# zju3dv/LoFTR

Hardware: AMD Instinct MI355X
Metric: image-pairs/sec @640x480 indoor-ds (higher is better)
Workload: dtype f32; 1 GPU; batch=8 640x480 synthetic grayscale pairs per GPU, indoor_ds dual-softmax (BASELINE configs[1]), full LoFTR.forward = ResNet-FPN backbone (HIP implicit-GEMM / patch convolutions incl. the 7x7 stem) + HIP matching path; weights=seeded random init (no checkpoint on the box), conf_matrix_materialised=True, match_type=dual_softmax, global_batch=8, parallelism=dp1 (pairs sharded; RCCL all-gather of match counts)

## Files before the change

loftr_amd/csrc/common.h:

```cpp
#pragma once
#include <hip/hip_runtime.h>
#include <stdint.h>
#include <stddef.h>
#include "../../include/loftr_hip.h"

typedef float f32x16 __attribute__((ext_vector_type(16)));
typedef float f32x4 __attribute__((ext_vector_type(4)));
typedef float f32x2 __attribute__((ext_vector_type(2)));

#define LOFTR_NEG_INF (-1e9f)

#define LOFTR_CHECK_ARG(cond) do { if (!(cond)) return LOFTR_ERR_BAD_ARG; } while (0)
#define LOFTR_CHECK_LAUNCH() do { if (hipGetLastError() != hipSuccess) return LOFTR_ERR_LAUNCH; } while (0)

#ifdef __HIP_DEVICE_COMPILE__
#define LOFTR_NO_PACKED_FP32 __attribute__((target("no-packed-fp32-ops")))
#else
#define LOFTR_NO_PACKED_FP32
#endif

__host__ __device__ static inline int ceil_div(int a, int b) { return (a + b - 1) / b; }
static inline size_t align_up(size_t x, size_t a) { return (x + a - 1) / a * a; }

enum LoftrTimedKernel {
// ... 13 lines not shown
  LOFTR_T_ENCODER_X = 13,
  LOFTR_T_FINE_PAIR = 14,
  LOFTR_T_COUNT = 15
};
enum LoftrDebugKey {
  LOFTR_DBG_ENCODER_SCHEDULE = 0,
  LOFTR_DBG_CONV_PERSIST_CAP,
  LOFTR_DBG_WGRAD_CHUNK,
  LOFTR_DBG_REDUCE_TALL,
  LOFTR_DBG_PCT_GRID,
  LOFTR_DBG_PCT_SKIP,
  LOFTR_DBG_PCT_QUOTA,
  LOFTR_DBG_CONV_DUO,
  LOFTR_DBG_CONV_PATCH,
  LOFTR_DBG_CONV_REM,
  LOFTR_DBG_COUNT
};
int loftr_debug_value(int key);
extern unsigned g_loftr_timing_mask;
extern int g_loftr_range_check;
void loftr_timing_mark(int id, hipStream_t st, bool end);
struct TimedLaunch {
  int id; hipStream_t st; bool on;
  TimedLaunch(int id_, hipStream_t st_) : id(id_), st(st_), on((g_loftr_timing_mask >> id_) & 1u) {
    if (on) loftr_timing_mark(id, st, false);
  }
  ~TimedLaunch() { if (on) loftr_timing_mark(id, st, true); }
};

constexpr int NUM_XCD = 8;
// ... 98 lines not shown
```

loftr_amd/csrc/fine_fused.hip:

```cpp
#include "linear.h"

#ifdef LOFTR_FINE_PROBE
__device__ long long* g_fine_probe = nullptr;
#define FFX_STAMP(i_) { const long long t__ = wall_clock64(); pacc[i_] += t__ - pt__; pt__ = t__; }
#else
#define FFX_STAMP(i_)
#endif
#ifndef FFX_PROBE_READS
#define FFX_PROBE_READS 1
#endif
#ifndef FFX_PROBE_DMA
#define FFX_PROBE_DMA 1
#endif
#ifndef FFX_PROBE_BARRIER
#define FFX_PROBE_BARRIER 1
#endif
namespace {
namespace ffx {
constexpr int W = 4, STAGE = 16 * 1024, BLK = 4096, NST = 6, DMA_PER_WAVE = 4;
constexpr int PPC = 8 + 8 + 24, NCALL = 4, NPANEL = PPC * NCALL;
constexpr int T_QS = 0, T_KS = 128, T_VS = 256, T_MS = 384, T_W0S = 512, T_W2S = 768, T_G1 = 896, T_B1 = 1024, T_G2 = 1152,
              T_B2 = 1280, T_LAYER = 1408;
constexpr int OFF_TAB = NST * STAGE, OFF_KSUM = OFF_TAB + 2 * T_LAYER * 4;
constexpr int OFF_KV = OFF_KSUM + W * 512;
constexpr int OFF_DESC = OFF_KV + W * 8192;
constexpr int LDS_BYTES = OFF_DESC + NPANEL * 16;
static_assert(LDS_BYTES <= 160 * 1024, "one workgroup per CU");

struct Args {
  float* f0; float* f1;
  int M, T;
  const sp_t* wq[2]; const sp_t* wk[2]; const sp_t* wv[2]; const sp_t* wm[2]; const sp_t* w0[2]; const sp_t* w2[2];
  const float* sq[2]; const float* sk[2]; const float* sv[2]; const float* sm[2]; const float* s0[2]; const float* s2[2];
  const float* g1[2]; const float* b1[2]; const float* g2[2]; const float* b2[2];
  float attn_eps, ln_eps;
};

typedef __attribute__((address_space(3))) void* lds_ptr_t;
typedef const __attribute__((address_space(1))) void* gbl_ptr_t;

__device__ __forceinline__ void swap_halves(uint32_t& a, uint32_t& b) {
  const auto r = __builtin_amdgcn_permlane32_swap(a, b, false, false);
// ... 39 lines not shown
__device__ __forceinline__ float wave_absmax16(const float (&v)[16]) {
  float m = 0.f;
#pragma unroll
  for (int r = 0; r < 16; ++r) m = fmaxf(m, fabsf(v[r]));
  m = half_max(m);
  return fmaxf(m, swap32(m));
}
__device__ __forceinline__ void pack8(const float (&v)[8], h16x8& fh, h16x8& fl) {
  uint32_t hi[4], lo[4];
#pragma unroll
  for (int e = 0; e < 4; ++e) sp_pack2(v[2 * e], v[2 * e + 1], hi[e], lo[e]);
  fh = __builtin_bit_cast(h16x8, u32x4{hi[0], hi[1], hi[2], hi[3]});
  fl = __builtin_bit_cast(h16x8, u32x4{lo[0], lo[1], lo[2], lo[3]});
}

__device__ __forceinline__ float kv_tile(const f32x16& kacc, const f32x16& vacc, float ksc, float vsc, int T, int g, int li,
                                         unsigned ksum_ad, unsigned kv_ad) {
  float kk[16], vv[16], ksum = 0.f;
#pragma unroll
  for (int r = 0; r < 16; ++r) {
    const bool ok = (r & 3) + 8 * (r >> 2) + 4 * g < T;
    const float kx = kacc[r] * ksc;
    kk[r] = ok ? (kx > 0.f ? kx + 1.f : __expf(kx)) : 0.f;
    vv[r] = ok ? vacc[r] * vsc : 0.f;
    ksum += kk[r];
  }
  ksum += swap32(ksum);
  float v_inv;
  const float v_sc = pow2_lift(wave_absmax16(vv), v_inv);
#pragma unroll
// ... 18 lines not shown
  }
  float kvv[16];
#pragma unroll
  for (int r = 0; r < 16; ++r) kvv[r] = kv[r];
  float kv_inv;
  const float kv_sc = pow2_lift(wave_absmax16(kvv), kv_inv);
#pragma unroll
  for (int r = 0; r < 16; ++r) kvv[r] *= kv_sc;
  h16x8 fh[2], fl[2];
  pack_panel(kvv, fh, fl);
  const u32x4 mh = __builtin_bit_cast(u32x4, li < 16 ? fh[0] : fh[1]), ml = __builtin_bit_cast(u32x4, li < 16 ? fl[0] : fl[1]);
  asm volatile("ds_write_b128 %0, %1\n\tds_write_b128 %0, %2 offset:1024" :: "v"(kv_ad), "v"(mh), "v"(ml) : "memory");
  return v_inv * kv_inv;
}

__global__ __launch_bounds__(W * 64, 1) void fine_pair_kernel(Args a) {
  __shared__ __attribute__((aligned(16))) char lds[LDS_BYTES];
  const int lane = threadIdx.x & 63, wave = threadIdx.x >> 6, g = lane >> 5, li = lane & 31;
  const int T = a.T;
  const long m = (long)blockIdx.x * W + wave;
  const bool live = m < a.M;
  const long mc = live ? m : a.M - 1;
  float* tab = reinterpret_cast<float*>(lds + OFF_TAB);
  const unsigned ksum_addr = (unsigned)(size_t)(lds_ptr_t)(lds + OFF_KSUM + wave * 512);
  const float* ksum_tab = reinterpret_cast<const float*>(lds + OFF_KSUM + wave * 512);
  const unsigned kv_addr = (unsigned)(size_t)(lds_ptr_t)(lds + OFF_KV + wave * 8192);
  const char* kv_tab = lds + OFF_KV + wave * 8192 + lane * 16;

  for (int f = threadIdx.x; f < 256; f += W * 64) {
#pragma unroll
    for (int l = 0; l < 2; ++l) {
      float* tl = tab + l * T_LAYER;
      tl[T_W0S + f] = a.s0[l][f];
      if (f < 128) {
        tl[T_QS + f] = a.sq[l][f]; tl[T_KS + f] = a.sk[l][f]; tl[T_VS + f] = a.sv[l][f]; tl[T_MS + f] = a.sm[l][f];
        tl[T_W2S + f] = a.s2[l][f];
        tl[T_G1 + f] = a.g1[l][f]; tl[T_B1 + f] = a.b1[l][f]; tl[T_G2 + f] = a.g2[l][f]; tl[T_B2 + f] = a.b2[l][f];
      }
    }
  }
  h16x8 wah[8], wal[8], wbh[8], wbl[8];
  float wa_sc, wa_inv, wb_sc, wb_inv;
  {
    const long row = (mc * T + min(li, T - 1)) * 128;
    const f32x4* p0 = reinterpret_cast<const f32x4*>(a.f0 + row);
    const f32x4* p1 = reinterpret_cast<const f32x4*>(a.f1 + row);
    f32x4 ua[16], ub[16];
    float ma = 0.f, mb = 0.f;
#pragma unroll
    for (int i = 0; i < 16; ++i) {
      ua[i] = p0[4 * (i >> 1) + 2 * g + (i & 1)]; ub[i] = p1[4 * (i >> 1) + 2 * g + (i & 1)];
#pragma unroll
      for (int e = 0; e < 4; ++e) { ma = fmaxf(ma, fabsf(ua[i][e])); mb = fmaxf(mb, fabsf(ub[i][e])); }
    }
    ma = half_max(ma); ma = fmaxf(ma, swap32(ma)); mb = half_max(mb); mb = fmaxf(mb, swap32(mb));
    wa_sc = pow2_lift(ma, wa_inv); wb_sc = pow2_lift(mb, wb_inv);
#pragma unroll
    for (int ks = 0; ks < 8; ++ks) {
      const f32x4 u0 = ua[2 * ks] * wa_sc, u1 = ua[2 * ks + 1] * wa_sc, v0 = ub[2 * ks] * wb_sc, v1 = ub[2 * ks + 1] * wb_sc;
      const float xa[8] = {u0[0], u0[1], u0[2], u0[3], u1[0], u1[1], u1[2], u1[3]};
      const float xb[8] = {v0[0], v0[1], v0[2], v0[3], v1[0], v1[1], v1[2], v1[3]};
      pack8(xa, wah[ks], wal[ks]);
      pack8(xb, wbh[ks], wbl[ks]);
    }
  }

  unsigned off128[4];
#pragma unroll
  for (int oct = 0; oct < 4; ++oct) {
    const unsigned ro = oct * 8 + (lane >> 3), ch = ((lane & 7) ^ ((oct * 4 + (lane >> 4)) & 7)) << 2;
    off128[oct] = (ro * 128 + ch) * 4;
  }
  const unsigned rl512 = (unsigned)(lane >> 3) * 512u;
  const int wave_s = __builtin_amdgcn_readfirstlane(wave);
  for (int p = threadIdx.x; p < NPANEL; p += W * 64) {
    const int c = p / PPC, q = p - c * PPC, l = c >> 1;
    int off, pitch = 128, mat, kt = 0;
    if (q < 8) { mat = (q & 1) ? 2 : 1; off = (q >> 1) * 32 * 128; }
    else if (q < 16) { const int t = (q - 8) >> 1; if (q & 1) { mat = 3; off = t * 32; kt = 1; } else { mat = 0; off = t * 32 * 128; } }
    else { const int hp = (q - 16) / 3, i = (q - 16) - 3 * hp; pitch = 256;
           if (i == 2) { mat = 5; off = hp * 32; kt = 1; } else { mat = 4; off = hp * 32 * 256 + i * 128; } }
    const sp_t* mp = mat == 0 ? a.wq[l] : mat == 1 ? a.wk[l] : mat == 2 ? a.wv[l] : mat == 3 ? a.wm[l] : mat == 4 ? a.w0[l] : a.w2[l];
    const unsigned long long ad = (unsigned long long)(size_t)(mp + off);
    reinterpret_cast<int4*>(lds + OFF_DESC)[p] = make_int4((int)(unsigned)ad, (int)(unsigned)(ad >> 32), pitch, kt);
  }
#define FFX_ISSUE(p_)                                                                                      \
  {                                                                                                        \
    const int p__ = (p_);                                                                                  \
    const int4 d__ = reinterpret_cast<const int4*>(lds + OFF_DESC)[p__];                                   \
    const unsigned lo__ = (unsigned)__builtin_amdgcn_readfirstlane(d__.x), hi__ = (unsigned)__builtin_amdgcn_readfirstlane(d__.y); \
    const int pitch__ = __builtin_amdgcn_readfirstlane(d__.z), kt__ = __builtin_amdgcn_readfirstlane(d__.w);        \
    const unsigned long long wo__ = (unsigned long long)(kt__ ? wave_s * 32 * pitch__ : wave_s * 32) * 4ull;    \
    const char* base__ = reinterpret_cast<const char*>((size_t)((((unsigned long long)hi__ << 32) | lo__) + wo__)); \
    char* st__ = lds + (p__ % NST) * STAGE + wave_s * BLK;                                                 \
    const unsigned w256__ = pitch__ == 256 ? 1u : 0u;                                                      \
    _Pragma("unroll") for (int oct__ = 0; oct__ < 4; ++oct__)                                              \
      __builtin_amdgcn_global_load_lds((gbl_ptr_t)(base__ + (size_t)(w256__ * (unsigned)(oct__ * 4096)) + (off128[oct__] + w256__ * rl512)), \
                                       (lds_ptr_t)(st__ + oct__ * 1024), 16, 0, 0);                        \
  }
#define FFX_BEGIN(p_)                                                                                      \
  {                                                                                                        \
    const int rem__ = NPANEL - 1 - (p_);                                                                   \
    if (!FFX_PROBE_DMA) LOFTR_WAITCNT_VM(0);                                                               \
    else if (rem__ >= 4) LOFTR_WAITCNT_VM(4 * DMA_PER_WAVE);                                                    \
    else if (rem__ == 3) LOFTR_WAITCNT_VM(3 * DMA_PER_WAVE);                                               \
    else if (rem__ == 2) LOFTR_WAITCNT_VM(2 * DMA_PER_WAVE);                                               \
    else if (rem__ == 1) LOFTR_WAITCNT_VM(1 * DMA_PER_WAVE);                                               \
    else LOFTR_WAITCNT_VM(0);                                                                              \
    if (FFX_PROBE_BARRIER) __builtin_amdgcn_s_barrier();                                                   \
    if (FFX_PROBE_DMA && (p_) + NST - 1 < NPANEL) FFX_ISSUE((p_) + NST - 1);                                                \
  }
  const int a_off = lds_chunk_off(li, g);
#define FFX_RD(st_, blk_, odd_, lo_) (*reinterpret_cast<const h16x8*>((st_) + (blk_) * BLK + (a_off ^ (((odd_) ? 32 : 0) | ((lo_) ? 64 : 0)))))
#define FFX_USE(a_, b_, c_, d_) asm volatile("" :: "v"(a_), "v"(b_), "v"(c_), "v"(d_))
#define FFX_UNITS(st_, BLK0_, ODD0_, BLK1_, ODD1_, M1_, M2_, M3_, M4_, M5_, M6_)                           \
  {                                                                                                        \
    h16x8 ah__ = FFX_RD(st_, BLK0_(0), ODD0_(0), 0), al__ = FFX_RD(st_, BLK0_(0), ODD0_(0), 1);            \
    h16x8 bh__ = FFX_RD(st_, BLK1_(0), ODD1_(0), 0), bl__ = FFX_RD(st_, BLK1_(0), ODD1_(0), 1);            \
    _Pragma("unroll") for (int u = 0; u < 4; ++u) {                                                        \
      FFX_USE(ah__, al__, bh__, bl__);                                                                     \
      __builtin_amdgcn_sched_barrier(0);                                                                   \
      h16x8 nah__ = ah__, nal__ = al__, nbh__ = bh__, nbl__ = bl__;                                        \
      M1_;                                                                                                 \
      __builtin_amdgcn_sched_barrier(0);                                                                   \
      if (FFX_PROBE_READS && u + 1 < 4) { nah__ = FFX_RD(st_, BLK0_(u + 1), ODD0_(u + 1), 0); nal__ = FFX_RD(st_, BLK0_(u + 1), ODD0_(u + 1), 1); } \
      __builtin_amdgcn_sched_barrier(0);                                                                   \
      M2_;                                                                                                 \
      __builtin_amdgcn_sched_barrier(0);                                                                   \
      if (FFX_PROBE_READS && u + 1 < 4) { nbh__ = FFX_RD(st_, BLK1_(u + 1), ODD1_(u + 1), 0); nbl__ = FFX_RD(st_, BLK1_(u + 1), ODD1_(u + 1), 1); } \
      __builtin_amdgcn_sched_barrier(0);                                                                   \
      M3_; M4_; M5_; M6_;                                                                                  \
      __builtin_amdgcn_sched_barrier(0);                                                                   \
      ah__ = nah__; al__ = nal__; bh__ = nbh__; bl__ = nbl__;                                              \
    }                                                                                                      \
  }
#define FFX_MF(A_, B_, C_) C_ = __builtin_amdgcn_mfma_f32_32x32x16_f16(A_, B_, C_, 0, 0, 0)
#define FFX_ID(u_) (u_)
#define FFX_ZERO(u_) 0
#define FFX_ONE(u_) 1
#define FFX_RPANEL(st_, xh_, xl_, acc_)                                                                    \
  FFX_UNITS(st_, FFX_ID, FFX_ZERO, FFX_ID, FFX_ONE,                                                        \
            FFX_MF(ah__, xl_[2 * u], acc_), FFX_MF(al__, xh_[2 * u], acc_), FFX_MF(ah__, xh_[2 * u], acc_), \
            FFX_MF(bh__, xl_[2 * u + 1], acc_), FFX_MF(bl__, xh_[2 * u + 1], acc_), FFX_MF(bh__, xh_[2 * u + 1], acc_))
#define FFX_TPANEL(st_, xh_, xl_, acc_)                                                                    \
  FFX_UNITS(st_, FFX_ID, FFX_ZERO, FFX_ID, FFX_ONE,                                                        \
            FFX_MF(xh_[2 * u], al__, acc_), FFX_MF(xl_[2 * u], ah__, acc_), FFX_MF(xh_[2 * u], ah__, acc_), \
            FFX_MF(xh_[2 * u + 1], bl__, acc_), FFX_MF(xl_[2 * u + 1], bh__, acc_), FFX_MF(xh_[2 * u + 1], bh__, acc_))
#define FFX_KB0(u_) (2 * ((u_) >> 1))
#define FFX_KB1(u_) (2 * ((u_) >> 1) + 1)
#define FFX_KODD(u_) ((u_) & 1)
#define FFX_KPANEL(st_, fh_, fl_, out_)                                                                    \
  FFX_UNITS(st_, FFX_KB0, FFX_KODD, FFX_KB1, FFX_KODD,                                                     \
            FFX_MF(ah__, fl_[u & 1], out_[2 * (u >> 1)]), FFX_MF(bh__, fl_[u & 1], out_[2 * (u >> 1) + 1]), \
            FFX_MF(al__, fh_[u & 1], out_[2 * (u >> 1)]), FFX_MF(bl__, fh_[u & 1], out_[2 * (u >> 1) + 1]), \
            FFX_MF(ah__, fh_[u & 1], out_[2 * (u >> 1)]), FFX_MF(bh__, fh_[u & 1], out_[2 * (u >> 1) + 1]))

  LOFTR_WAITCNT_VM(0);
  __syncthreads();
#pragma unroll
  for (int p = 0; p < NST - 1; ++p) FFX_ISSUE(p);

#ifdef LOFTR_FINE_PROBE
  long long pacc[8] = {0, 0, 0, 0, 0, 0, 0, 0};
  const long long pstart__ = wall_clock64();
  long long pt__ = pstart__;
#endif
  const int fq = 4 * g;
  const float S = (float)T, inv_s = 1.f / (float)T;
  const h16x8 zero8 = __builtin_bit_cast(h16x8, u32x4{0u, 0u, 0u, 0u});
  f32x16 acc, acc2;
  f32x16 big[4];

#pragma unroll 1
  for (int c = 0; c < NCALL; ++c) {
    const int p0 = c * PPC;
    const float* tl = tab + (c >> 1) * T_LAYER;
    const bool self = c < 2;
    const float src_sc = self ? wa_sc : wb_sc, src_inv = self ? wa_inv : wb_inv;
    float kvi[4] = {1.f, 1.f, 1.f, 1.f};
#define FFX_KV_LOOP(SH_, SL_)                                                                              \
    _Pragma("unroll 1") for (int t = 0; t < 4; ++t) {                                                      \
      const int p = p0 + 2 * t;                                                                            \
      FFX_BEGIN(p);                                                                                        \
      if (live) {                                                                                          \
        _Pragma("unroll") for (int r = 0; r < 16; ++r) acc[r] = 0.f;                                       \
        FFX_TPANEL(lds + (p % NST) * STAGE, SH_, SL_, acc);        \
      }                                                                                                    \
      FFX_BEGIN(p + 1);                                                                                    \
      if (live) {                                                                                          \
        _Pragma("unroll") for (int r = 0; r < 16; ++r) acc2[r] = 0.f;                                      \
        FFX_TPANEL(lds + ((p + 1) % NST) * STAGE, SH_, SL_, acc2);                             \
        const float inv__ = kv_tile(acc, acc2, tl[T_KS + 32 * t + li] * src_inv, tl[T_VS + 32 * t + li] * inv_s * src_inv, T, g, li, \
                                    ksum_addr + (unsigned)((32 * t + li) * 4), kv_addr + (unsigned)(t * 2048 + lane * 16));  \
        kvi[0] = kvi[1]; kvi[1] = kvi[2]; kvi[2] = kvi[3]; kvi[3] = inv__;                                 \
      }                                                                                                    \
    }
    FFX_STAMP(0)
    if (self) { FFX_KV_LOOP(wah, wal) } else { FFX_KV_LOOP(wbh, wbl) }
#undef FFX_KV_LOOP
    FFX_STAMP(1)
    asm volatile("s_waitcnt lgkmcnt(0)" ::: "memory");
#pragma unroll
    for (int j = 0; j < 4; ++j)
#pragma unroll
      for (int r = 0; r < 16; ++r) big[j][r] = 0.f;
#pragma unroll 1
    for (int t = 0; t < 4; ++t) {
      const int p = p0 + 8 + 2 * t;
      FFX_BEGIN(p);
      h16x8 mah[2], mal[2];
      if (live) {
#pragma unroll
        for (int r = 0; r < 16; ++r) acc[r] = 0.f;
        FFX_RPANEL(lds + (p % NST) * STAGE, wah, wal, acc);
        float v[16], den0 = 0.f, den1 = 0.f;
#pragma unroll
        for (int q = 0; q < 4; ++q) {
          const f32x4 ws = *reinterpret_cast<const f32x4*>(tl + T_QS + 32 * t + fq + 8 * q);
          const f32x4 ks4 = *reinterpret_cast<const f32x4*>(ksum_tab + 32 * t + fq + 8 * q);
#pragma unroll
          for (int e = 0; e < 4; ++e) {
            float x = acc[4 * q + e] * (ws[e] * wa_inv);
            x = x > 0.f ? x + 1.f : __expf(x);
            v[4 * q + e] = x;
            if (q < 2) den0 = fmaf(x, ks4[e], den0); else den1 = fmaf(x, ks4[e], den1);
          }
        }
        den0 += swap32(den0); den1 += swap32(den1);
        const float z0 = S * __builtin_amdgcn_rcpf(den0 + a.attn_eps), z1 = S * __builtin_amdgcn_rcpf(den1 + a.attn_eps);
// ... 11 lines not shown
        const h16x8 kvh0 = *reinterpret_cast<const h16x8*>(kv_tab + t * 2048), kvl0 = *reinterpret_cast<const h16x8*>(kv_tab + t * 2048 + 1024);
        const h16x8 a0h = li < 16 ? kvh0 : zero8, a0l = li < 16 ? kvl0 : zero8;
        const h16x8 a1h = li < 16 ? zero8 : kvh0, a1l = li < 16 ? zero8 : kvl0;
        f32x16 at;
#pragma unroll
        for (int r = 0; r < 16; ++r) at[r] = 0.f;
        FFX_MF(a0h, ql[0], at); FFX_MF(a0l, qh[0], at); FFX_MF(a0h, qh[0], at);
        FFX_MF(a1h, ql[1], at); FFX_MF(a1l, qh[1], at); FFX_MF(a1h, qh[1], at);
        kvi[0] = kvi[1]; kvi[1] = kvi[2]; kvi[2] = kvi[3];
        float av[16];
#pragma unroll
        for (int r = 0; r < 16; ++r) av[r] = at[r] * undo;
        pack_panel(av, mah, mal);
      }
      FFX_BEGIN(p + 1);
      if (live) FFX_KPANEL(lds + ((p + 1) % NST) * STAGE, mah, mal, big);
    }
    FFX_STAMP(2)
    h16x8 mh[8], ml[8];
    if (live) {
      float s = 0.f;
#pragma unroll
      for (int j = 0; j < 4; ++j)
#pragma unroll
        for (int q = 0; q < 4; ++q) {
          const f32x4 ws = *reinterpret_cast<const f32x4*>(tl + T_MS + 32 * j + fq + 8 * q);
#pragma unroll
          for (int e = 0; e < 4; ++e) { big[j][4 * q + e] *= ws[e] * (4.f * src_inv); s += big[j][4 * q + e]; }
        }
      s += swap32(s);
      const float mean = s * (1.f / 128.f);
      float m2 = 0.f;
#pragma unroll
      for (int j = 0; j < 4; ++j)
#pragma unroll
        for (int r = 0; r < 16; ++r) { const float d = big[j][r] - mean; m2 = fmaf(d, d, m2); }
      m2 += swap32(m2);
      const float rstd = rsqrtf(m2 * (1.f / 128.f) + a.ln_eps);
#pragma unroll
      for (int j = 0; j < 4; ++j) {
        float y[16];
#pragma unroll
        for (int q = 0; q < 4; ++q) {
          const f32x4 ga = *reinterpret_cast<const f32x4*>(tl + T_G1 + 32 * j + fq + 8 * q);
          const f32x4 be = *reinterpret_cast<const f32x4*>(tl + T_B1 + 32 * j + fq + 8 * q);
#pragma unroll
          for (int e = 0; e < 4; ++e) y[4 * q + e] = (big[j][4 * q + e] - mean) * rstd * ga[e] + be[e];
        }
        h16x8 fh[2], fl[2];
        pack_panel(y, fh, fl);
        mh[2 * j] = fh[0]; mh[2 * j + 1] = fh[1]; ml[2 * j] = fl[0]; ml[2 * j + 1] = fl[1];
      }
    }
#pragma unroll
    for (int j = 0; j < 4; ++j)
#pragma unroll
      for (int r = 0; r < 16; ++r) big[j][r] = 0.f;
    FFX_STAMP(3)
#pragma unroll 1
    for (int hp = 0; hp < 8; ++hp) {
      const int p = p0 + 16 + 3 * hp;
      h16x8 hh[2], hl[2];
      FFX_BEGIN(p);
      if (live) {
#pragma unroll
        for (int r = 0; r < 16; ++r) acc[r] = 0.f;
        FFX_RPANEL(lds + (p % NST) * STAGE, wah, wal, acc);
      }
      FFX_BEGIN(p + 1);
      if (live) {
#pragma unroll
        for (int r = 0; r < 16; ++r) acc2[r] = 0.f;
        FFX_RPANEL(lds + ((p + 1) % NST) * STAGE, mh, ml, acc2);
        float v[16];
#pragma unroll
        for (int q = 0; q < 4; ++q) {
          const f32x4 ws = *reinterpret_cast<const f32x4*>(tl + T_W0S + 32 * hp + fq + 8 * q);
#pragma unroll
          for (int e = 0; e < 4; ++e) v[4 * q + e] = fmaxf(fmaf(acc[4 * q + e], wa_inv, acc2[4 * q + e]) * ws[e], 0.f);
        }
        pack_panel(v, hh, hl);
      }
      FFX_BEGIN(p + 2);
      if (live) FFX_KPANEL(lds + ((p + 2) % NST) * STAGE, hh, hl, big);
    }
    FFX_STAMP(4)
    if (live) {
      float* orow = ((c & 1) ? a.f1 : a.f0) + (mc * T + min(li, T - 1)) * 128;
      f32x4 xres[16];
#pragma unroll
      for (int j = 0; j < 4; ++j)
#pragma unroll
        for (int q = 0; q < 4; ++q) xres[4 * j + q] = *reinterpret_cast<const f32x4*>(orow + 32 * j + fq + 8 * q);
      float s = 0.f;
#pragma unroll
      for (int j = 0; j < 4; ++j)
#pragma unroll
        for (int q = 0; q < 4; ++q) {
          const f32x4 ws = *reinterpret_cast<const f32x4*>(tl + T_W2S + 32 * j + fq + 8 * q);
#pragma unroll
          for (int e = 0; e < 4; ++e) { big[j][4 * q + e] *= ws[e]; s += big[j][4 * q + e]; }
        }
      s += swap32(s);
      const float mean = s * (1.f / 128.f);
      float m2 = 0.f;
#pragma unroll
      for (int j = 0; j < 4; ++j)
#pragma unroll
        for (int r = 0; r < 16; ++r) { const float d = big[j][r] - mean; m2 = fmaf(d, d, m2); }
      m2 += swap32(m2);
      const float rstd = rsqrtf(m2 * (1.f / 128.f) + a.ln_eps);
      const bool store = li < T;
      float y[4][16], ym = 0.f;
#pragma unroll
      for (int j = 0; j < 4; ++j) {
#pragma unroll
        for (int q = 0; q < 4; ++q) {
          const f32x4 ga = *reinterpret_cast<const f32x4*>(tl + T_G2 + 32 * j + fq + 8 * q);
          const f32x4 be = *reinterpret_cast<const f32x4*>(tl + T_B2 + 32 * j + fq + 8 * q);
          f32x4 o;
#pragma unroll
          for (int e = 0; e < 4; ++e) {
            o[e] = xres[4 * j + q][e] + ((big[j][4 * q + e] - mean) * rstd * ga[e] + be[e]);
            y[j][4 * q + e] = o[e];
            ym = fmaxf(ym, fabsf(o[e]));
          }
          if (store) *reinterpret_cast<f32x4*>(orow + 32 * j + fq + 8 * q) = o;
        }
      }
      ym = half_max(ym); ym = fmaxf(ym, swap32(ym));
      wa_sc = pow2_lift(ym, wa_inv);
#pragma unroll
      for (int j = 0; j < 4; ++j) {
#pragma unroll
        for (int r = 0; r < 16; ++r) y[j][r] *= wa_sc;
        h16x8 fh[2], fl[2];
        pack_panel(y[j], fh, fl);
        wah[2 * j] = fh[0]; wah[2 * j + 1] = fh[1]; wal[2 * j] = fl[0]; wal[2 * j + 1] = fl[1];
      }
    }
#pragma unroll
    for (int ks = 0; ks < 8; ++ks) {
      const h16x8 th = wah[ks], tlo = wal[ks];
      wah[ks] = wbh[ks]; wal[ks] = wbl[ks]; wbh[ks] = th; wbl[ks] = tlo;
    }
    { const float ts = wa_sc, ti = wa_inv; wa_sc = wb_sc; wa_inv = wb_inv; wb_sc = ts; wb_inv = ti; }
    FFX_STAMP(5)
  }
#ifdef LOFTR_FINE_PROBE
  if (g_fine_probe && lane == 0) {
    long long* o = g_fine_probe + ((long)blockIdx.x * W + wave) * 8;
    for (int i = 0; i < 6; ++i) o[i] = pacc[i];
    o[6] = pstart__; o[7] = wall_clock64();
  }
#endif
#undef FFX_ISSUE
#undef FFX_BEGIN
#undef FFX_RD
#undef FFX_USE
#undef FFX_UNITS
#undef FFX_MF
#undef FFX_ID
#undef FFX_ZERO
#undef FFX_ONE
#undef FFX_RPANEL
#undef FFX_TPANEL
#undef FFX_KB0
#undef FFX_KB1
#undef FFX_KODD
#undef FFX_KPANEL
}
}
}

#ifdef LOFTR_FINE_PROBE
extern "C" int loftr_fine_probe_buffer(void* buf) {
  long long* b = (long long*)buf;
  return hipMemcpyToSymbol(HIP_SYMBOL(g_fine_probe), &b, sizeof(b)) == hipSuccess ? LOFTR_OK : LOFTR_ERR_LAUNCH;
}
#endif

int launch_fine_pair(const FinePairArgs& p, hipStream_t st) {
  if (p.C != 128 || p.T < 1 || p.T > 32 || p.M <= 0) return LOFTR_ERR_UNSUPPORTED;
  ffx::Args a{};
  a.f0 = p.f0; a.f1 = p.f1; a.M = p.M; a.T = p.T; a.attn_eps = p.attn_eps; a.ln_eps = p.ln_eps;
  for (int l = 0; l < 2; ++l) {
    a.wq[l] = p.wq[l]; a.wk[l] = p.wk[l]; a.wv[l] = p.wv[l]; a.wm[l] = p.wm[l]; a.w0[l] = p.w0[l]; a.w2[l] = p.w2[l];
    a.sq[l] = p.sq[l]; a.sk[l] = p.sk[l]; a.sv[l] = p.sv[l]; a.sm[l] = p.sm[l]; a.s0[l] = p.s0[l]; a.s2[l] = p.s2[l];
    a.g1[l] = p.g1[l]; a.b1[l] = p.b1[l]; a.g2[l] = p.g2[l]; a.b2[l] = p.b2[l];
    if (!a.wq[l] || !a.sq[l] || !a.sk[l] || !a.sv[l] || !a.sm[l] || !a.s0[l] || !a.s2[l]) return LOFTR_ERR_UNSUPPORTED;
  }
  TimedLaunch tl(LOFTR_T_FINE_PAIR, st);
  hipLaunchKernelGGL(ffx::fine_pair_kernel, dim3(ceil_div(p.M, ffx::W)), dim3(ffx::W * 64), 0, st, a);
  LOFTR_CHECK_LAUNCH();
  return LOFTR_OK;
}
```

loftr_amd/csrc/misc.hip:

```cpp
#include "common.h"
#include <string.h>

namespace {
template <bool CL>
__global__ void pos_encode_flatten_kernel(loftr_fmap f, const float* __restrict__ pe,
                                          int pe_h, int pe_w, float* __restrict__ out, int C) {
  __shared__ float tile[32][33];
  const int H = f.H, W = f.W, HW = H * W;
  const int n = blockIdx.z, hw0 = blockIdx.x * 32, c0 = blockIdx.y * 32;
  const float* in = f.data + (long)n * f.sn;
  for (int k = threadIdx.y; k < 32; k += 8) {
    const int c = c0 + k, hw = hw0 + threadIdx.x;
    float v = 0.f;
    if (c < C && hw < HW) {
      const int y = hw / W, x = hw - y * W;
      v = pe[((long)c * pe_h + y) * pe_w + x];
      if (!CL) v += in[(long)c * f.sc + (long)y * f.sh + (long)x * f.sw];
    }
    tile[k][threadIdx.x] = v;
  }
  __syncthreads();
  for (int k = threadIdx.y; k < 32; k += 8) {
    const int hw = hw0 + k, c = c0 + threadIdx.x;
    if (hw < HW && c < C) {
// ... 10 lines not shown
  LOFTR_CHECK_ARG(feat && feat->data && pe && out && N >= 0 && C > 0 && feat->H > 0 && feat->W > 0 &&
                  feat->H <= pe_h && feat->W <= pe_w);
  if (N == 0) return LOFTR_OK;
  const dim3 grid(ceil_div(feat->H * feat->W, 32), ceil_div(C, 32), N), block(32, 8);
  if (feat->sc == 1)
    hipLaunchKernelGGL((pos_encode_flatten_kernel<true>), grid, block, 0, (hipStream_t)stream, *feat, pe, pe_h, pe_w, out, C);
  else
    hipLaunchKernelGGL((pos_encode_flatten_kernel<false>), grid, block, 0, (hipStream_t)stream, *feat, pe, pe_h, pe_w, out, C);
  LOFTR_CHECK_LAUNCH();
  return LOFTR_OK;
}

namespace {
struct DebugSwitch { const char* name; int def; int value; };
DebugSwitch g_debug[LOFTR_DBG_COUNT] = {{"encoder_schedule", 1, 1}, {"conv_persist_cap", 0, 0}, {"wgrad_chunk", 0, 0}, {"reduce_tall", 1, 1},
                                        {"pct_grid", 0, 0}, {"pct_skip", 0, 0}, {"pct_quota", 0, 0}, {"conv_duo", 1, 1}, {"conv_patch", 1, 1}, {"conv_rem", 1, 1}};
}
int loftr_debug_value(int key) { return (key >= 0 && key < LOFTR_DBG_COUNT) ? g_debug[key].value : 0; }
extern "C" int loftr_hip_debug_set(const char* key, int value) {
  LOFTR_CHECK_ARG(key != nullptr);
  for (auto& d : g_debug)
    if (strcmp(d.name, key) == 0) { d.value = value; return LOFTR_OK; }
  return LOFTR_ERR_BAD_ARG;
}
extern "C" int loftr_hip_debug_get(const char* key, int* value, int* default_value) {
  LOFTR_CHECK_ARG(key != nullptr && value != nullptr);
  for (auto& d : g_debug)
    if (strcmp(d.name, key) == 0) { *value = d.value; if (default_value) *default_value = d.def; return LOFTR_OK; }
  return LOFTR_ERR_BAD_ARG;
}

// ... 88 lines not shown
```

Baseline: 455.9 image-pairs/s.

## Add 8-wave fine_pair_kernel variant with shared panel DMA and reloaded windows

Templates the fused fine-matching kernel on wave count, adding an 8-wave configuration (4 LDS stages, half the DMA issues per wave, no register prefetch, low-half of FFN input stashed in LDS) picked when M is large. Window features are now reloaded from global memory per call instead of being held and rescaled in registers across layers. Dead waves now run the maths and only skip the store. The aim is more waves per CU to hide latency and less register pressure, at the cost of extra global reloads, LDS traffic and scheduling barriers.

```diff
diff --git a/loftr_amd/csrc/common.h b/loftr_amd/csrc/common.h
--- a/loftr_amd/csrc/common.h
+++ b/loftr_amd/csrc/common.h
@@ -51,6 +51,7 @@
   LOFTR_DBG_CONV_DUO,
   LOFTR_DBG_CONV_PATCH,
   LOFTR_DBG_CONV_REM,
+  LOFTR_DBG_FINE_WAVES,
   LOFTR_DBG_COUNT
 };
 int loftr_debug_value(int key);
diff --git a/loftr_amd/csrc/fine_fused.hip b/loftr_amd/csrc/fine_fused.hip
--- a/loftr_amd/csrc/fine_fused.hip
+++ b/loftr_amd/csrc/fine_fused.hip
@@ -15,17 +15,26 @@
 #ifndef FFX_PROBE_BARRIER
 #define FFX_PROBE_BARRIER 1
 #endif
+#ifndef FFX_PRIO_HALF
+#define FFX_PRIO_HALF 0
+#endif
 namespace {
 namespace ffx {
-constexpr int W = 4, STAGE = 16 * 1024, BLK = 4096, NST = 6, DMA_PER_WAVE = 4;
+constexpr int STAGE = 16 * 1024, BLK = 4096;
 constexpr int PPC = 8 + 8 + 24, NCALL = 4, NPANEL = PPC * NCALL;
 constexpr int T_QS = 0, T_KS = 128, T_VS = 256, T_MS = 384, T_W0S = 512, T_W2S = 768, T_G1 = 896, T_B1 = 1024, T_G2 = 1152,
               T_B2 = 1280, T_LAYER = 1408;
-constexpr int OFF_TAB = NST * STAGE, OFF_KSUM = OFF_TAB + 2 * T_LAYER * 4;
-constexpr int OFF_KV = OFF_KSUM + W * 512;
-constexpr int OFF_DESC = OFF_KV + W * 8192;
-constexpr int LDS_BYTES = OFF_DESC + NPANEL * 16;
-static_assert(LDS_BYTES <= 160 * 1024, "one workgroup per CU");
+template <int W> struct Geo {
+  static constexpr int NST = W == 4 ? 6 : 4;
+  static constexpr int DMA_PER_WAVE = 16 / W;
+  static constexpr bool PREFETCH = W == 4;
+  static constexpr bool STASH = W == 8;
+  static constexpr int OFF_TAB = NST * STAGE, OFF_KSUM = OFF_TAB + 2 * T_LAYER * 4;
+  static constexpr int OFF_KV = OFF_KSUM + W * 512;
+  static constexpr int OFF_DESC = OFF_KV + W * 8192;
+  static constexpr int LDS_BYTES = OFF_DESC + NPANEL * 16;
+  static_assert(NST >= 3 && NST <= 6 && LDS_BYTES <= 160 * 1024, "one workgroup per CU");
+};
 
 struct Args {
   float* f0; float* f1;
@@ -95,6 +104,26 @@
   fl = __builtin_bit_cast(h16x8, u32x4{lo[0], lo[1], lo[2], lo[3]});
 }
 
+__device__ __forceinline__ void load_window(const float* win, unsigned off, h16x8 (&fh)[8], h16x8 (&fl)[8], float& sc, float& inv) {
+  const f32x4* p = reinterpret_cast<const f32x4*>(reinterpret_cast<const char*>(win) + off);
+  f32x4 u[16];
+  float m = 0.f;
+#pragma unroll
+  for (int i = 0; i < 16; ++i) {
+    u[i] = p[4 * (i >> 1) + (i & 1)];
+#pragma unroll
+    for (int e = 0; e < 4; ++e) m = fmaxf(m, fabsf(u[i][e]));
+  }
+  m = half_max(m); m = fmaxf(m, swap32(m));
+  sc = pow2_lift(m, inv);
+#pragma unroll
+  for (int ks = 0; ks < 8; ++ks) {
+    const f32x4 u0 = u[2 * ks] * sc, u1 = u[2 * ks + 1] * sc;
+    const float x[8] = {u0[0], u0[1], u0[2], u0[3], u1[0], u1[1], u1[2], u1[3]};
+    pack8(x, fh[ks], fl[ks]);
+  }
+}
+
 __device__ __forceinline__ float kv_tile(const f32x16& kacc, const f32x16& vacc, float ksc, float vsc, int T, int g, int li,
                                          unsigned ksum_ad, unsigned kv_ad) {
   float kk[16], vv[16], ksum = 0.f;
@@ -143,18 +172,24 @@
   return v_inv * kv_inv;
 }
 
+template <int W>
 __global__ __launch_bounds__(W * 64, 1) void fine_pair_kernel(Args a) {
-  __shared__ __attribute__((aligned(16))) char lds[LDS_BYTES];
+  using G = Geo<W>;
+  constexpr int NST = G::NST, DMA_PER_WAVE = G::DMA_PER_WAVE, OFF_TAB = G::OFF_TAB, OFF_KSUM = G::OFF_KSUM, OFF_KV = G::OFF_KV,
+                OFF_DESC = G::OFF_DESC;
+  constexpr bool PREFETCH = G::PREFETCH, STASH = G::STASH;
+  __shared__ __attribute__((aligned(16))) char lds[G::LDS_BYTES];
   const int lane = threadIdx.x & 63, wave = threadIdx.x >> 6, g = lane >> 5, li = lane & 31;
   const int T = a.T;
-  const long m = (long)blockIdx.x * W + wave;
-  const bool live = m < a.M;
-  const long mc = live ? m : a.M - 1;
+  const int wave_s = __builtin_amdgcn_readfirstlane(wave);
+  const long m = (long)blockIdx.x * W + wave_s;
+  const bool owner = m < a.M;
+  const long mc = owner ? m : a.M - 1;
   float* tab = reinterpret_cast<float*>(lds + OFF_TAB);
-  const unsigned ksum_addr = (unsigned)(size_t)(lds_ptr_t)(lds + OFF_KSUM + wave * 512);
-  const float* ksum_tab = reinterpret_cast<const float*>(lds + OFF_KSUM + wave * 512);
-  const unsigned kv_addr = (unsigned)(size_t)(lds_ptr_t)(lds + OFF_KV + wave * 8192);
-  const char* kv_tab = lds + OFF_KV + wave * 8192 + lane * 16;
+  const unsigned ksum_addr = (unsigned)(size_t)(lds_ptr_t)(lds + OFF_KSUM + wave_s * 512);
+  const float* ksum_tab = reinterpret_cast<const float*>(lds + OFF_KSUM + wave_s * 512);
+  const unsigned kv_addr = (unsigned)(size_t)(lds_ptr_t)(lds + OFF_KV + wave_s * 8192);
+  const char* kv_tab = lds + OFF_KV + wave_s * 8192 + lane * 16;
 
   for (int f = threadIdx.x; f < 256; f += W * 64) {
 #pragma unroll
@@ -168,40 +203,18 @@
       }
     }
   }
-  h16x8 wah[8], wal[8], wbh[8], wbl[8];
-  float wa_sc, wa_inv, wb_sc, wb_inv;
-  {
-    const long row = (mc * T + min(li, T - 1)) * 128;
-    const f32x4* p0 = reinterpret_cast<const f32x4*>(a.f0 + row);
-    const f32x4* p1 = reinterpret_cast<const f32x4*>(a.f1 + row);
-    f32x4 ua[16], ub[16];
-    float ma = 0.f, mb = 0.f;
-#pragma unroll
-    for (int i = 0; i < 16; ++i) {
-      ua[i] = p0[4 * (i >> 1) + 2 * g + (i & 1)]; ub[i] = p1[4 * (i >> 1) + 2 * g + (i & 1)];
-#pragma unroll
-      for (int e = 0; e < 4; ++e) { ma = fmaxf(ma, fabsf(ua[i][e])); mb = fmaxf(mb, fabsf(ub[i][e])); }
-    }
-    ma = half_max(ma); ma = fmaxf(ma, swap32(ma)); mb = half_max(mb); mb = fmaxf(mb, swap32(mb));
-    wa_sc = pow2_lift(ma, wa_inv); wb_sc = pow2_lift(mb, wb_inv);
-#pragma unroll
-    for (int ks = 0; ks < 8; ++ks) {
-      const f32x4 u0 = ua[2 * ks] * wa_sc, u1 = ua[2 * ks + 1] * wa_sc, v0 = ub[2 * ks] * wb_sc, v1 = ub[2 * ks + 1] * wb_sc;
-      const float xa[8] = {u0[0], u0[1], u0[2], u0[3], u1[0], u1[1], u1[2], u1[3]};
-      const float xb[8] = {v0[0], v0[1], v0[2], v0[3], v1[0], v1[1], v1[2], v1[3]};
-      pack8(xa, wah[ks], wal[ks]);
-      pack8(xb, wbh[ks], wbl[ks]);
-    }
-  }
-
-  unsigned off128[4];
-#pragma unroll
-  for (int oct = 0; oct < 4; ++oct) {
+  float* const f0m = a.f0 + mc * T * 128;
+  float* const f1m = a.f1 + mc * T * 128;
+  const unsigned rowoff = (unsigned)min(li, T - 1) * 512u;
+  const int blk_s = (wave_s * DMA_PER_WAVE) >> 2, oct_s = (wave_s * DMA_PER_WAVE) & 3;
+  unsigned off128[DMA_PER_WAVE];
+#pragma unroll
+  for (int i = 0; i < DMA_PER_WAVE; ++i) {
+    const unsigned oct = oct_s + i;
     const unsigned ro = oct * 8 + (lane >> 3), ch = ((lane & 7) ^ ((oct * 4 + (lane >> 4)) & 7)) << 2;
-    off128[oct] = (ro * 128 + ch) * 4;
+    off128[i] = (ro * 128 + ch) * 4;
   }
   const unsigned rl512 = (unsigned)(lane >> 3) * 512u;
-  const int wave_s = __builtin_amdgcn_readfirstlane(wave);
   for (int p = threadIdx.x; p < NPANEL; p += W * 64) {
     const int c = p / PPC, q = p - c * PPC, l = c >> 1;
     int off, pitch = 128, mat, kt = 0;
@@ -219,19 +232,19 @@
     const int4 d__ = reinterpret_cast<const int4*>(lds + OFF_DESC)[p__];                                   \
     const unsigned lo__ = (unsigned)__builtin_amdgcn_readfirstlane(d__.x), hi__ = (unsigned)__builtin_amdgcn_readfirstlane(d__.y); \
     const int pitch__ = __builtin_amdgcn_readfirstlane(d__.z), kt__ = __builtin_amdgcn_readfirstlane(d__.w);        \
-    const unsigned long long wo__ = (unsigned long long)(kt__ ? wave_s * 32 * pitch__ : wave_s * 32) * 4ull;    \
+    const unsigned long long wo__ = (unsigned long long)(kt__ ? blk_s * 32 * pitch__ : blk_s * 32) * 4ull;    \
     const char* base__ = reinterpret_cast<const char*>((size_t)((((unsigned long long)hi__ << 32) | lo__) + wo__)); \
-    char* st__ = lds + (p__ % NST) * STAGE + wave_s * BLK;                                                 \
+    char* st__ = lds + (p__ % NST) * STAGE + blk_s * BLK + oct_s * 1024;                                   \
     const unsigned w256__ = pitch__ == 256 ? 1u : 0u;                                                      \
-    _Pragma("unroll") for (int oct__ = 0; oct__ < 4; ++oct__)                                              \
-      __builtin_amdgcn_global_load_lds((gbl_ptr_t)(base__ + (size_t)(w256__ * (unsigned)(oct__ * 4096)) + (off128[oct__] + w256__ * rl512)), \
-                                       (lds_ptr_t)(st__ + oct__ * 1024), 16, 0, 0);                        \
+    _Pragma("unroll") for (int i__ = 0; i__ < DMA_PER_WAVE; ++i__)                                         \
+      __builtin_amdgcn_global_load_lds((gbl_ptr_t)(base__ + (size_t)(w256__ * (unsigned)((oct_s + i__) * 4096)) + (off128[i__] + w256__ * rl512)), \
+                                       (lds_ptr_t)(st__ + i__ * 1024), 16, 0, 0);                          \
   }
 #define FFX_BEGIN(p_)                                                                                      \
   {                                                                                                        \
-    const int rem__ = NPANEL - 1 - (p_);                                                                   \
+    const int rem__ = min(NPANEL - 1 - (p_), NST - 2);                         \
     if (!FFX_PROBE_DMA) LOFTR_WAITCNT_VM(0);                                                               \
-    else if (rem__ >= 4) LOFTR_WAITCNT_VM(4 * DMA_PER_WAVE);                                                    \
+    else if (rem__ == 4) LOFTR_WAITCNT_VM(4 * DMA_PER_WAVE);                                               \
     else if (rem__ == 3) LOFTR_WAITCNT_VM(3 * DMA_PER_WAVE);                                               \
     else if (rem__ == 2) LOFTR_WAITCNT_VM(2 * DMA_PER_WAVE);                                               \
     else if (rem__ == 1) LOFTR_WAITCNT_VM(1 * DMA_PER_WAVE);                                               \
@@ -242,7 +255,7 @@
   const int a_off = lds_chunk_off(li, g);
 #define FFX_RD(st_, blk_, odd_, lo_) (*reinterpret_cast<const h16x8*>((st_) + (blk_) * BLK + (a_off ^ (((odd_) ? 32 : 0) | ((lo_) ? 64 : 0)))))
 #define FFX_USE(a_, b_, c_, d_) asm volatile("" :: "v"(a_), "v"(b_), "v"(c_), "v"(d_))
-#define FFX_UNITS(st_, BLK0_, ODD0_, BLK1_, ODD1_, M1_, M2_, M3_, M4_, M5_, M6_)                           \
+#define FFX_UNITS_P(st_, BLK0_, ODD0_, BLK1_, ODD1_, M1_, M2_, M3_, M4_, M5_, M6_)                         \
   {                                                                                                        \
     h16x8 ah__ = FFX_RD(st_, BLK0_(0), ODD0_(0), 0), al__ = FFX_RD(st_, BLK0_(0), ODD0_(0), 1);            \
     h16x8 bh__ = FFX_RD(st_, BLK1_(0), ODD1_(0), 0), bl__ = FFX_RD(st_, BLK1_(0), ODD1_(0), 1);            \
@@ -263,29 +276,49 @@
       ah__ = nah__; al__ = nal__; bh__ = nbh__; bl__ = nbl__;                                              \
     }                                                                                                      \
   }
+#define FFX_UNITS_NP(st_, BLK0_, ODD0_, BLK1_, ODD1_, AB_, M1_, M2_, M3_, M4_, M5_, M6_)                   \
+  _Pragma("unroll") for (int u = 0; u < 4; ++u) {                                                          \
+    h16x8 ah__, al__, bh__, bl__;                                                                          \
+    __builtin_amdgcn_sched_barrier(0);                                                                     \
+    ah__ = FFX_RD(st_, BLK0_(u), ODD0_(u), 0); al__ = FFX_RD(st_, BLK0_(u), ODD0_(u), 1);                  \
+    if (AB_) { M1_; M2_; M3_; __builtin_amdgcn_sched_barrier(0); }                                         \
+    bh__ = FFX_RD(st_, BLK1_(u), ODD1_(u), 0); bl__ = FFX_RD(st_, BLK1_(u), ODD1_(u), 1);                  \
+    if (!(AB_)) { M1_; M2_; M3_; }                                                                         \
+    M4_; M5_; M6_;                                                                                         \
+    __builtin_amdgcn_sched_barrier(0);                                                                     \
+  }
+#define FFX_UNITS(st_, BLK0_, ODD0_, BLK1_, ODD1_, AB_, M1_, M2_, M3_, M4_, M5_, M6_)                      \
+  {                                                                                                        \
+    if (PREFETCH) FFX_UNITS_P(st_, BLK0_, ODD0_, BLK1_, ODD1_, M1_, M2_, M3_, M4_, M5_, M6_)               \
+    else FFX_UNITS_NP(st_, BLK0_, ODD0_, BLK1_, ODD1_, AB_, M1_, M2_, M3_, M4_, M5_, M6_)                  \
+  }
+#define FFX_AFTER(x_, DEP_) { if (!PREFETCH) asm volatile("" : "+v"(x_) : "v"(DEP_)); }
 #define FFX_MF(A_, B_, C_) C_ = __builtin_amdgcn_mfma_f32_32x32x16_f16(A_, B_, C_, 0, 0, 0)
 #define FFX_ID(u_) (u_)
 #define FFX_ZERO(u_) 0
 #define FFX_ONE(u_) 1
-#define FFX_RPANEL(st_, xh_, xl_, acc_)                                                                    \
-  FFX_UNITS(st_, FFX_ID, FFX_ZERO, FFX_ID, FFX_ONE,                                                        \
-            FFX_MF(ah__, xl_[2 * u], acc_), FFX_MF(al__, xh_[2 * u], acc_), FFX_MF(ah__, xh_[2 * u], acc_), \
-            FFX_MF(bh__, xl_[2 * u + 1], acc_), FFX_MF(bl__, xh_[2 * u + 1], acc_), FFX_MF(bh__, xh_[2 * u + 1], acc_))
+#define FFX_RPANEL(st_, xh_, XL_, acc_)                                                                    \
+  FFX_UNITS(st_, FFX_ID, FFX_ZERO, FFX_ID, FFX_ONE, 1,                                                      \
+            FFX_MF(ah__, XL_(2 * u), acc_), FFX_MF(al__, xh_[2 * u], acc_), FFX_MF(ah__, xh_[2 * u], acc_), \
+            FFX_MF(bh__, XL_(2 * u + 1), acc_), FFX_MF(bl__, xh_[2 * u + 1], acc_), FFX_MF(bh__, xh_[2 * u + 1], acc_))
+#define FFX_XL(k_) xl[k_]
+#define FFX_ML(k_) (STASH ? *reinterpret_cast<const h16x8*>(kv_tab + (k_) * 1024) : ml[k_])
 #define FFX_TPANEL(st_, xh_, xl_, acc_)                                                                    \
-  FFX_UNITS(st_, FFX_ID, FFX_ZERO, FFX_ID, FFX_ONE,                                                        \
+  FFX_UNITS(st_, FFX_ID, FFX_ZERO, FFX_ID, FFX_ONE, 1,                                                      \
             FFX_MF(xh_[2 * u], al__, acc_), FFX_MF(xl_[2 * u], ah__, acc_), FFX_MF(xh_[2 * u], ah__, acc_), \
             FFX_MF(xh_[2 * u + 1], bl__, acc_), FFX_MF(xl_[2 * u + 1], bh__, acc_), FFX_MF(xh_[2 * u + 1], bh__, acc_))
 #define FFX_KB0(u_) (2 * ((u_) >> 1))
 #define FFX_KB1(u_) (2 * ((u_) >> 1) + 1)
 #define FFX_KODD(u_) ((u_) & 1)
 #define FFX_KPANEL(st_, fh_, fl_, out_)                                                                    \
-  FFX_UNITS(st_, FFX_KB0, FFX_KODD, FFX_KB1, FFX_KODD,                                                     \
+  FFX_UNITS(st_, FFX_KB0, FFX_KODD, FFX_KB1, FFX_KODD, 0,                                                   \
             FFX_MF(ah__, fl_[u & 1], out_[2 * (u >> 1)]), FFX_MF(bh__, fl_[u & 1], out_[2 * (u >> 1) + 1]), \
             FFX_MF(al__, fh_[u & 1], out_[2 * (u >> 1)]), FFX_MF(bl__, fh_[u & 1], out_[2 * (u >> 1) + 1]), \
             FFX_MF(ah__, fh_[u & 1], out_[2 * (u >> 1)]), FFX_MF(bh__, fh_[u & 1], out_[2 * (u >> 1) + 1]))
 
   LOFTR_WAITCNT_VM(0);
   __syncthreads();
+  if (FFX_PRIO_HALF && W == 8 && wave_s >= 4) __builtin_amdgcn_s_setprio(1);
 #pragma unroll
   for (int p = 0; p < NST - 1; ++p) FFX_ISSUE(p);
 
@@ -297,7 +330,6 @@
   const int fq = 4 * g;
   const float S = (float)T, inv_s = 1.f / (float)T;
   const h16x8 zero8 = __builtin_bit_cast(h16x8, u32x4{0u, 0u, 0u, 0u});
-  f32x16 acc, acc2;
   f32x16 big[4];
 
 #pragma unroll 1
@@ -305,18 +337,25 @@
     const int p0 = c * PPC;
     const float* tl = tab + (c >> 1) * T_LAYER;
     const bool self = c < 2;
-    const float src_sc = self ? wa_sc : wb_sc, src_inv = self ? wa_inv : wb_inv;
+    float* xwin = (c & 1) ? f1m : f0m;
+    const float* swin = ((c & 1) != 0) == self ? f1m : f0m;
+    float src_sc = 1.f, src_inv = 1.f, wa_sc = 1.f, wa_inv = 1.f;
+    h16x8 xh[8], xl[8];
+    f32x16 acc, acc2;
+    __builtin_amdgcn_fence(__ATOMIC_ACQ_REL, "wavefront");
+    if (!self) LOFTR_WAITCNT_VM(0);
+    load_window(swin, rowoff + 32u * g, xh, xl, src_sc, src_inv);
     float kvi[4] = {1.f, 1.f, 1.f, 1.f};
 #define FFX_KV_LOOP(SH_, SL_)                                                                              \
     _Pragma("unroll 1") for (int t = 0; t < 4; ++t) {                                                      \
       const int p = p0 + 2 * t;                                                                            \
       FFX_BEGIN(p);                                                                                        \
-      if (live) {                                                                                          \
+      {                                                                                                    \
         _Pragma("unroll") for (int r = 0; r < 16; ++r) acc[r] = 0.f;                                       \
         FFX_TPANEL(lds + (p % NST) * STAGE, SH_, SL_, acc);        \
       }                                                                                                    \
       FFX_BEGIN(p + 1);                                                                                    \
-      if (live) {                                                                                          \
+      {                                                                                                    \
         _Pragma("unroll") for (int r = 0; r < 16; ++r) acc2[r] = 0.f;                                      \
         FFX_TPANEL(lds + ((p + 1) % NST) * STAGE, SH_, SL_, acc2);                             \
         const float inv__ = kv_tile(acc, acc2, tl[T_KS + 32 * t + li] * src_inv, tl[T_VS + 32 * t + li] * inv_s * src_inv, T, g, li, \
@@ -325,10 +364,12 @@
       }                                                                                                    \
     }
     FFX_STAMP(0)
-    if (self) { FFX_KV_LOOP(wah, wal) } else { FFX_KV_LOOP(wbh, wbl) }
+    FFX_KV_LOOP(xh, xl)
 #undef FFX_KV_LOOP
     FFX_STAMP(1)
     asm volatile("s_waitcnt lgkmcnt(0)" ::: "memory");
+    wa_sc = src_sc; wa_inv = src_inv;
+    if (!self) load_window(xwin, rowoff + 32u * g, xh, xl, wa_sc, wa_inv);
 #pragma unroll
     for (int j = 0; j < 4; ++j)
 #pragma unroll
@@ -338,10 +379,10 @@
       const int p = p0 + 8 + 2 * t;
       FFX_BEGIN(p);
       h16x8 mah[2], mal[2];
-      if (live) {
+      {
 #pragma unroll
         for (int r = 0; r < 16; ++r) acc[r] = 0.f;
-        FFX_RPANEL(lds + (p % NST) * STAGE, wah, wal, acc);
+        FFX_RPANEL(lds + (p % NST) * STAGE, xh, FFX_XL, acc);
         float v[16], den0 = 0.f, den1 = 0.f;
 #pragma unroll
         for (int q = 0; q < 4; ++q) {
@@ -383,17 +424,19 @@
         pack_panel(av, mah, mal);
       }
       FFX_BEGIN(p + 1);
-      if (live) FFX_KPANEL(lds + ((p + 1) % NST) * STAGE, mah, mal, big);
+      FFX_KPANEL(lds + ((p + 1) % NST) * STAGE, mah, mal, big);
     }
     FFX_STAMP(2)
     h16x8 mh[8], ml[8];
-    if (live) {
+    {
       float s = 0.f;
+      int fqs = fq;
 #pragma unroll
       for (int j = 0; j < 4; ++j)
 #pragma unroll
         for (int q = 0; q < 4; ++q) {
-          const f32x4 ws = *reinterpret_cast<const f32x4*>(tl + T_MS + 32 * j + fq + 8 * q);
+          if (q == 0) FFX_AFTER(fqs, s)
+          const f32x4 ws = *reinterpret_cast<const f32x4*>(tl + T_MS + 32 * j + fqs + 8 * q);
 #pragma unroll
           for (int e = 0; e < 4; ++e) { big[j][4 * q + e] *= ws[e] * (4.f * src_inv); s += big[j][4 * q + e]; }
         }
@@ -409,17 +452,25 @@
 #pragma unroll
       for (int j = 0; j < 4; ++j) {
         float y[16];
+        if (j > 0) FFX_AFTER(fqs, mh[2 * j - 1])
 #pragma unroll
         for (int q = 0; q < 4; ++q) {
-          const f32x4 ga = *reinterpret_cast<const f32x4*>(tl + T_G1 + 32 * j + fq + 8 * q);
-          const f32x4 be = *reinterpret_cast<const f32x4*>(tl + T_B1 + 32 * j + fq + 8 * q);
+          const f32x4 ga = *reinterpret_cast<const f32x4*>(tl + T_G1 + 32 * j + fqs + 8 * q);
+          const f32x4 be = *reinterpret_cast<const f32x4*>(tl + T_B1 + 32 * j + fqs + 8 * q);
 #pragma unroll
           for (int e = 0; e < 4; ++e) y[4 * q + e] = (big[j][4 * q + e] - mean) * rstd * ga[e] + be[e];
         }
         h16x8 fh[2], fl[2];
         pack_panel(y, fh, fl);
-        mh[2 * j] = fh[0]; mh[2 * j + 1] = fh[1]; ml[2 * j] = fl[0]; ml[2 * j + 1] = fl[1];
+        mh[2 * j] = fh[0]; mh[2 * j + 1] = fh[1];
+        if (STASH) {
+          const u32x4 l0 = __builtin_bit_cast(u32x4, fl[0]), l1 = __builtin_bit_cast(u32x4, fl[1]);
+          asm volatile("ds_write_b128 %0, %1\n\tds_write_b128 %0, %2 offset:1024" :: "v"(kv_addr + (unsigned)(j * 2048 + lane * 16)), "v"(l0), "v"(l1) : "memory");
+        } else {
+          ml[2 * j] = fl[0]; ml[2 * j + 1] = fl[1];
+        }
       }
+      if (STASH) asm volatile("s_waitcnt lgkmcnt(0)" ::: "memory");
     }
 #pragma unroll
     for (int j = 0; j < 4; ++j)
@@ -431,16 +482,16 @@
       const int p = p0 + 16 + 3 * hp;
       h16x8 hh[2], hl[2];
       FFX_BEGIN(p);
-      if (live) {
+      {
 #pragma unroll
         for (int r = 0; r < 16; ++r) acc[r] = 0.f;
-        FFX_RPANEL(lds + (p % NST) * STAGE, wah, wal, acc);
+        FFX_RPANEL(lds + (p % NST) * STAGE, xh, FFX_XL, acc);
       }
       FFX_BEGIN(p + 1);
-      if (live) {
+      {
 #pragma unroll
         for (int r = 0; r < 16; ++r) acc2[r] = 0.f;
-        FFX_RPANEL(lds + ((p + 1) % NST) * STAGE, mh, ml, acc2);
+        FFX_RPANEL(lds + ((p + 1) % NST) * STAGE, mh, FFX_ML, acc2);
         float v[16];
 #pragma unroll
         for (int q = 0; q < 4; ++q) {
@@ -451,16 +502,16 @@
         pack_panel(v, hh, hl);
       }
       FFX_BEGIN(p + 2);
-      if (live) FFX_KPANEL(lds + ((p + 2) % NST) * STAGE, hh, hl, big);
+      FFX_KPANEL(lds + ((p + 2) % NST) * STAGE, hh, hl, big);
     }
     FFX_STAMP(4)
-    if (live) {
-      float* orow = ((c & 1) ? a.f1 : a.f0) + (mc * T + min(li, T - 1)) * 128;
+    {
+      float* orow = reinterpret_cast<float*>(reinterpret_cast<char*>(xwin) + (rowoff + 4u * fq));
       f32x4 xres[16];
 #pragma unroll
       for (int j = 0; j < 4; ++j)
 #pragma unroll
-        for (int q = 0; q < 4; ++q) xres[4 * j + q] = *reinterpret_cast<const f32x4*>(orow + 32 * j + fq + 8 * q);
+        for (int q = 0; q < 4; ++q) xres[4 * j + q] = *reinterpret_cast<const f32x4*>(orow + 32 * j + 8 * q);
       float s = 0.f;
 #pragma unroll
       for (int j = 0; j < 4; ++j)
@@ -479,8 +530,7 @@
         for (int r = 0; r < 16; ++r) { const float d = big[j][r] - mean; m2 = fmaf(d, d, m2); }
       m2 += swap32(m2);
       const float rstd = rsqrtf(m2 * (1.f / 128.f) + a.ln_eps);
-      const bool store = li < T;
-      float y[4][16], ym = 0.f;
+      const bool store = li < T && owner;
 #pragma unroll
       for (int j = 0; j < 4; ++j) {
 #pragma unroll
@@ -489,31 +539,11 @@
           const f32x4 be = *reinterpret_cast<const f32x4*>(tl + T_B2 + 32 * j + fq + 8 * q);
           f32x4 o;
 #pragma unroll
-          for (int e = 0; e < 4; ++e) {
-            o[e] = xres[4 * j + q][e] + ((big[j][4 * q + e] - mean) * rstd * ga[e] + be[e]);
-            y[j][4 * q + e] = o[e];
-            ym = fmaxf(ym, fabsf(o[e]));
-          }
-          if (store) *reinterpret_cast<f32x4*>(orow + 32 * j + fq + 8 * q) = o;
+          for (int e = 0; e < 4; ++e) o[e] = xres[4 * j + q][e] + ((big[j][4 * q + e] - mean) * rstd * ga[e] + be[e]);
+          if (store) *reinterpret_cast<f32x4*>(orow + 32 * j + 8 * q) = o;
         }
       }
-      ym = half_max(ym); ym = fmaxf(ym, swap32(ym));
-      wa_sc = pow2_lift(ym, wa_inv);
-#pragma unroll
-      for (int j = 0; j < 4; ++j) {
-#pragma unroll
-        for (int r = 0; r < 16; ++r) y[j][r] *= wa_sc;
-        h16x8 fh[2], fl[2];
-        pack_panel(y[j], fh, fl);
-        wah[2 * j] = fh[0]; wah[2 * j + 1] = fh[1]; wal[2 * j] = fl[0]; wal[2 * j + 1] = fl[1];
-      }
     }
-#pragma unroll
-    for (int ks = 0; ks < 8; ++ks) {
-      const h16x8 th = wah[ks], tlo = wal[ks];
-      wah[ks] = wbh[ks]; wal[ks] = wbl[ks]; wbh[ks] = th; wbl[ks] = tlo;
-    }
-    { const float ts = wa_sc, ti = wa_inv; wa_sc = wb_sc; wa_inv = wb_inv; wb_sc = ts; wb_inv = ti; }
     FFX_STAMP(5)
   }
 #ifdef LOFTR_FINE_PROBE
@@ -528,11 +558,16 @@
 #undef FFX_RD
 #undef FFX_USE
 #undef FFX_UNITS
+#undef FFX_UNITS_P
+#undef FFX_UNITS_NP
 #undef FFX_MF
+#undef FFX_AFTER
 #undef FFX_ID
 #undef FFX_ZERO
 #undef FFX_ONE
 #undef FFX_RPANEL
+#undef FFX_XL
+#undef FFX_ML
 #undef FFX_TPANEL
 #undef FFX_KB0
 #undef FFX_KB1
@@ -548,6 +583,8 @@
   return hipMemcpyToSymbol(HIP_SYMBOL(g_fine_probe), &b, sizeof(b)) == hipSuccess ? LOFTR_OK : LOFTR_ERR_LAUNCH;
 }
 #endif
+
+constexpr int FINE_WAVES8_MIN_M = 4 * 256 + 1;
 
 int launch_fine_pair(const FinePairArgs& p, hipStream_t st) {
   if (p.C != 128 || p.T < 1 || p.T > 32 || p.M <= 0) return LOFTR_ERR_UNSUPPORTED;
@@ -559,8 +596,11 @@
     a.g1[l] = p.g1[l]; a.b1[l] = p.b1[l]; a.g2[l] = p.g2[l]; a.b2[l] = p.b2[l];
     if (!a.wq[l] || !a.sq[l] || !a.sk[l] || !a.sv[l] || !a.sm[l] || !a.s0[l] || !a.s2[l]) return LOFTR_ERR_UNSUPPORTED;
   }
+  const int forced = loftr_debug_value(LOFTR_DBG_FINE_WAVES);
+  const bool eight = forced == 8 || (forced != 4 && p.M >= FINE_WAVES8_MIN_M);
   TimedLaunch tl(LOFTR_T_FINE_PAIR, st);
-  hipLaunchKernelGGL(ffx::fine_pair_kernel, dim3(ceil_div(p.M, ffx::W)), dim3(ffx::W * 64), 0, st, a);
+  if (eight) hipLaunchKernelGGL(ffx::fine_pair_kernel<8>, dim3(ceil_div(p.M, 8)), dim3(8 * 64), 0, st, a);
+  else hipLaunchKernelGGL(ffx::fine_pair_kernel<4>, dim3(ceil_div(p.M, 4)), dim3(4 * 64), 0, st, a);
   LOFTR_CHECK_LAUNCH();
   return LOFTR_OK;
 }
diff --git a/loftr_amd/csrc/misc.hip b/loftr_amd/csrc/misc.hip
--- a/loftr_amd/csrc/misc.hip
+++ b/loftr_amd/csrc/misc.hip
@@ -48,7 +48,8 @@
 namespace {
 struct DebugSwitch { const char* name; int def; int value; };
 DebugSwitch g_debug[LOFTR_DBG_COUNT] = {{"encoder_schedule", 1, 1}, {"conv_persist_cap", 0, 0}, {"wgrad_chunk", 0, 0}, {"reduce_tall", 1, 1},
-                                        {"pct_grid", 0, 0}, {"pct_skip", 0, 0}, {"pct_quota", 0, 0}, {"conv_duo", 1, 1}, {"conv_patch", 1, 1}, {"conv_rem", 1, 1}};
+                                        {"pct_grid", 0, 0}, {"pct_skip", 0, 0}, {"pct_quota", 0, 0}, {"conv_duo", 1, 1}, {"conv_patch", 1, 1}, {"conv_rem", 1, 1},
+                                        {"fine_waves", 0, 0}};
 }
 int loftr_debug_value(int key) { return (key >= 0 && key < LOFTR_DBG_COUNT) ? g_debug[key].value : 0; }
 extern "C" int loftr_hip_debug_set(const char* key, int value) {
```

Result: faster. 464.6 image-pairs/s (median of 6 runs) (+1.9%).
